# egordm/tch-geometric

Measured on AMD Instinct MI355X. Metric: sampled edges/sec, neighbor_sampling_homogenous fanout [15,10] on RMAT-24, higher is better.
Workload: dtype int64

## Files before the change

include/tchgeo.h:

```cpp
#ifndef TCHGEO_H
#define TCHGEO_H

#include <stdint.h>

#ifdef __cplusplus
extern "C" {
#endif

#define TG_API __attribute__((visibility("default")))

#define TG_OK 0
#define TG_ERR_INVALID 1
#define TG_ERR_HIP 2
#define TG_ERR_UNSUPPORTED 3

#define TG_MAX_HOPS 8
#define TG_MAX_FANOUT 32

typedef struct {
    const int64_t *ptrs;
    const int64_t *indices;
    const double *weights;
    const int64_t *timestamps;
    int64_t n_major;
// ... 71 lines not shown

TG_API int tg_ns_homo_batched_form(const tg_graph *csc, int64_t n_batches, int64_t n_seeds, const int64_t *fanout,
                            int32_t n_hops, const tg_ns_config *cfg, const tg_ns_out *out, int64_t workspace_bytes,
                            int32_t mode, int32_t *form, int32_t *n_windows);

TG_API int tg_ns_homo_batched_pipeline(const tg_graph *csc, int64_t n_batches, int64_t n_seeds, const int64_t *fanout,
                                int32_t n_hops, const tg_ns_config *cfg, const tg_ns_out *out, int64_t workspace_bytes,
                                int32_t mode, int32_t *staged);

typedef struct {
    int64_t window_bytes;
    int32_t gather_blocks;
    int32_t gather_threads;
    int32_t emit_threads;
    int32_t direct_hop0;
    int32_t fuse_first_hops;
    int32_t fold_hist;
    int32_t emit_blocks;
    int32_t staged;
    int32_t stage_round_chunks;
    int32_t stage_gather_threads;
    int32_t stage_gather_blocks;
    int32_t stage_emit_threads;
    int32_t stage_parts;
    int32_t stage_part_min_batches;
    int32_t stage_sort_blocks;
    int32_t stage_fine;
    int32_t stage_concurrent;
    int32_t stage_split;
    int32_t stage_split_round_chunks;
    int32_t store_align64;
    int32_t stage_fine_sub_bits;
    int32_t stage_fine_blocks;
} tg_ns_win_tuning;
TG_API int tg_ns_win_tuning_get(tg_ns_win_tuning *t);
TG_API int tg_ns_win_tuning_set(const tg_ns_win_tuning *t);

TG_API int tg_ns_win_stage_timing(int32_t enable);
TG_API int tg_ns_win_stage_times(float *ms, char *names, int32_t cap, int32_t *n);

typedef struct {
    const int64_t *vertices;
    const int64_t *ids;
    const int64_t *call_ids;
    int64_t m;
    int64_t id_base;
    int32_t fanout;
    int32_t sampler;
    uint32_t rng_tag;
    uint32_t _reserved;
} tg_hop_in;

typedef struct {
    int64_t *cnt;
    int64_t *offsets;
    int64_t *neighbors;
    int64_t *edge_ptrs;
    int64_t *parents;
} tg_hop_out;

TG_API int tg_ns_hop_workspace_bytes(int64_t m, int64_t *bytes);
TG_API int tg_ns_hop(const tg_graph *csc, const tg_hop_in *in, const tg_rng *rng, const tg_hop_out *out,
                     void *workspace, int64_t workspace_bytes, void *stream);

typedef struct {
    int32_t filter_mode;
// ... 293 lines not shown
```

tch-geometric_amd/csrc/ns_homo_win.hip:

```cpp
#include <stdlib.h>

#include <algorithm>
#include <mutex>

#include "ns_tickets.h"
#include "stage_bits.h"
#include "tg_device.h"
#include "tg_host.h"

namespace tg {

constexpr int WIN_PART_BLOCKS = 512;
constexpr int WIN_PART_THREADS = 512;
constexpr int WIN_TILE = 4096;
constexpr int WIN_MAX_BUCKETS = 8192;
constexpr int WIN_MAX_ROWS = 1024;
constexpr int WIN_MAX_PARTS = 16;

struct WinState {
    int64_t begin, end, ne, fbase;
};

struct WinQueues {
    struct alignas(256) Q {
// ... 8 lines not shown
    const uint32_t *ptrs32;
    const int64_t *seeds;
    int64_t n_seeds, n_batches;
    int32_t n_hops, hop, k, kmax;
    int64_t cap_nodes, cap_edges;
    int64_t *samples, *rows, *cols, *edge_index, *layer_offsets, *counts;
    uint64_t seed, call_id;
    uint32_t tag;
    int64_t id_base;
    WinState *state;
    CallKey *call_keys;
    unsigned long long *n_items;
    void *items_in, *items_sorted;
    uint32_t *hist;
    uint32_t *base;
    WinQueues *queues;
    int32_t n_buckets, shift;
    int32_t slot_bits;
    int32_t n_rows;
    int64_t item_pitch;
    uint32_t *vtab;
    uint32_t *stage;
    int32_t n_windows, idx_bits, next_idx_bits;
    int32_t n_wbuckets;
    uint32_t store_align;
    void *items_fine;
    uint16_t *item_keys;
    uint32_t *fine_rowtot;
    uint32_t *fine_tot, *fine_start;
    uint32_t *fine_tile_off;
    int64_t next_pitch;
    int64_t b0;
    int32_t fine_sub_bits;
    TG_BOUNDS_FIELDS
};

struct WinItemN {
    uint32_t e0, deg, bs, e;
    __device__ __forceinline__ static WinItemN make(uint64_t e0, uint32_t deg, uint32_t b, uint32_t slot, uint32_t e,
                                                    int slot_bits) {
        return WinItemN{(uint32_t)e0, deg, (b << slot_bits) | slot, e};
    }
    __device__ __forceinline__ uint64_t col() const { return e0; }
    __device__ __forceinline__ uint32_t batch(int slot_bits) const { return bs >> slot_bits; }
    __device__ __forceinline__ uint32_t slot(int slot_bits) const { return bs & ((1u << slot_bits) - 1u); }
};
struct WinItemW {
    uint64_t e0;
    uint32_t deg, b, s, e;
    __device__ __forceinline__ static WinItemW make(uint64_t e0, uint32_t deg, uint32_t b, uint32_t slot, uint32_t e,
                                                    int) {
        return WinItemW{e0, deg, b, slot, e};
    }
    __device__ __forceinline__ uint64_t col() const { return e0; }
    __device__ __forceinline__ uint32_t batch(int) const { return b; }
    __device__ __forceinline__ uint32_t slot(int) const { return s; }
};
static_assert(sizeof(WinItemN) == 16 && sizeof(WinItemW) == 24, "item layouts");

__device__ __forceinline__ uint32_t win_bucket(uint64_t e0, int shift, int n_buckets) {
    const uint32_t w = (uint32_t)(e0 >> shift);
    return (w & 7u) * (uint32_t)(n_buckets >> 3) + (w >> 3);
}

__global__ void win_init_kernel(const WinParams p, int64_t n_batches) {
    const int64_t b = blockIdx.x;
    int64_t *samples = p.samples + b * p.cap_nodes;
    for (int64_t i = threadIdx.x; i < p.n_seeds; i += blockDim.x) samples[i] = p.seeds[b * p.n_seeds + i];
    if (threadIdx.x == 0) {
        p.state[b] = WinState{0, p.n_seeds, 0, 0};
        p.call_keys[b] = call_key(p.seed, p.call_id + (uint64_t)b, p.tag);
        if (p.n_hops == 0) {
            p.counts[b * 2 + 0] = p.n_seeds;
            p.counts[b * 2 + 1] = 0;
        }
        if (b == 0)
            for (int h = 0; h < TG_MAX_HOPS; ++h) p.n_items[h] = 0ull;
    }
}

constexpr int WIN_ROUND_CHUNKS = 32;
constexpr int WIN_EMIT_MAX_THREADS = 512;
constexpr int WIN_STAGE_FIRST_RC = 16;
constexpr int WIN_STAGE_SIDE_RC = 8;

__host__ __device__ inline size_t win_emit_wave_lds_bytes(int kmax) {
    return (size_t)64 * kmax * sizeof(uint32_t) + (((size_t)64 * kmax + 15) & ~(size_t)15) + 64;
}

__host__ __device__ inline size_t win_emit_head_bytes(int rc = WIN_ROUND_CHUNKS) {
    return (((size_t)(rc + 1) * sizeof(uint32_t) + 15) & ~(size_t)15) + 16 +
           (size_t)rc * 64 * (sizeof(int64_t) + sizeof(uint32_t));
}
__host__ __device__ inline size_t win_emit_lds_bytes(int kmax, int n_waves, int rc = WIN_ROUND_CHUNKS) {
    return win_emit_head_bytes(rc) + (size_t)n_waves * win_emit_wave_lds_bytes(kmax);
}

__device__ __forceinline__ void win_next_item(const WinParams &p, int64_t b, uint32_t rel, uint32_t v, uint32_t *lhist);

template <typename Item, int KMAX, bool REPLACE, bool DIRECT, bool FOLD = false, bool NEXT = false, bool ITEMS = true,
          int RC = WIN_ROUND_CHUNKS>
__device__ __forceinline__ WinState win_emit_hop(const WinParams &p, unsigned char *smem, const int64_t b, const int hop,
                                                 const int k, const WinState st, const CallKey ck,
                                                 uint32_t *lhist = nullptr) {
    const int tid = threadIdx.x, lane = tid & 63, wave = tid >> 6, n_waves = blockDim.x >> 6;
    uint32_t *chunk_off = reinterpret_cast<uint32_t *>(smem);
    constexpr int64_t ROUND_SLOTS = (int64_t)RC * 64;
    const size_t off_bytes = (((size_t)(RC + 1) * sizeof(uint32_t)) + 15) & ~(size_t)15;
    int64_t *shared_fbase = reinterpret_cast<int64_t *>(smem + off_bytes);
    int64_t *col0 = reinterpret_cast<int64_t *>(smem + off_bytes + 16);
    uint32_t *cdeg = reinterpret_cast<uint32_t *>(smem + off_bytes + 16 + (size_t)ROUND_SLOTS * sizeof(int64_t));
    unsigned char *wbase = smem + win_emit_head_bytes(RC) + (size_t)wave * win_emit_wave_lds_bytes(p.kmax);
    uint32_t *spos = reinterpret_cast<uint32_t *>(wbase);
    uint8_t *slane = wbase + (size_t)64 * p.kmax * sizeof(uint32_t);
    Item *items = static_cast<Item *>(p.items_in);

    int64_t *samples = p.samples + b * p.cap_nodes;
    int64_t *rows = p.rows + b * p.cap_edges;
    int64_t *cols = p.cols + b * p.cap_edges;
    int64_t *eidx = p.edge_index + b * p.cap_edges;
    const int64_t n_seeds = p.n_seeds;
    const int64_t begin = st.begin, end = st.end;
    int64_t ne = st.ne;

    if (tid == 0) {
        int64_t *lo = p.layer_offsets + (b * p.n_hops + hop) * 3;
        lo[0] = n_seeds + ne;
        lo[1] = ne;
        lo[2] = n_seeds + ne;
        if (!FOLD) *shared_fbase = (DIRECT || !ITEMS) ? 0 : (int64_t)atomicAdd(&p.n_items[hop], (unsigned long long)(end - begin));
    }
    if (!FOLD) __syncthreads();
    const int64_t fbase = FOLD ? b * p.item_pitch : *shared_fbase;

    for (int64_t round_begin = begin; round_begin < end; round_begin += ROUND_SLOTS) {
        const int64_t round_end = min(end, round_begin + ROUND_SLOTS);
        const int nc = (int)((round_end - round_begin + 63) >> 6);
        for (int c = wave; c < nc; c += n_waves) {
            const int64_t i = round_begin + (int64_t)c * 64 + lane;
            int64_t e0 = 0, deg = 0;
            if (i < round_end) {
                int64_t w = samples[i];
                TG_CHECK_VERTEX(p, w);
                if (p.ptrs32) {
                    e0 = (int64_t)p.ptrs32[w];
                    deg = (int64_t)p.ptrs32[w + 1] - e0;
                } else {
                    e0 = p.ptrs[w];
                    deg = p.ptrs[w + 1] - e0;
                }
            }
            col0[c * 64 + lane] = e0;
            cdeg[c * 64 + lane] = deg > 0 ? (uint32_t)deg : 0u;
            const uint32_t cnt = (deg <= 0) ? 0u : (REPLACE ? (uint32_t)k : (uint32_t)min(deg, (int64_t)k));
            const uint32_t tot = wave_sum(cnt);
            if (lane == 0) chunk_off[c] = tot;
        }
        __syncthreads();
        if (wave == 0) {
            const uint32_t v = lane < nc ? chunk_off[lane] : 0u;
            const uint32_t incl = wave_inclusive_scan(v);
            if (lane < nc) chunk_off[lane] = incl - v;
            if (lane == 63) chunk_off[nc] = incl;
        }
        __syncthreads();
        for (int c = wave; c < nc; c += n_waves) {
            const int64_t i0 = round_begin + (int64_t)c * 64;
            const int64_t i = i0 + lane;
            const int64_t e0 = col0[c * 64 + lane];
            const uint32_t n = cdeg[c * 64 + lane];
            const uint32_t cnt = (n == 0) ? 0u : (REPLACE ? (uint32_t)k : min(n, (uint32_t)k));
            const uint64_t did = (uint64_t)(p.id_base + i);
            const uint32_t incl = wave_inclusive_scan(cnt);
            const uint32_t excl = incl - cnt;
            const uint32_t total = __shfl(incl, 63, 64);
            const int64_t e_chunk = ne + (int64_t)chunk_off[c];
            if (!DIRECT && ITEMS && i < round_end) {
                items[fbase + (i - begin)] =
                    Item::make((uint64_t)e0, n, (uint32_t)b, (uint32_t)i, (uint32_t)(e_chunk + excl), p.slot_bits);
                if (FOLD && n) atomicAdd(&lhist[win_bucket((uint64_t)e0, p.shift, p.n_buckets)], 1u);
            }
            const bool draws = REPLACE ? (cnt > 0) : (n > (uint32_t)k);
            const uint64_t dmask = __ballot(draws);
            const int n_draw = __popcll(dmask);
            const bool spread = n_draw > 0 && n_draw <= 32;
            if (spread) {
                uint8_t *dl = slane + (((size_t)64 * p.kmax + 15) & ~(size_t)15);
                const int my_rank = __popcll(dmask & ((lane == 0) ? 0ull : (~0ull >> (64 - lane))));
                if (draws) dl[my_rank] = (uint8_t)lane;
// ... 48 lines not shown
                    }
                } else {
                    sample_tickets<KMAX>(ck, did, n, k, spos, slane, excl, lane);
                }
            }
            wave_lds_handoff();
            if constexpr (DIRECT) {
                for (uint32_t q0 = 0; q0 < total; q0 += 256) {
                    int l4[4];
                    int64_t ep[4], v[4];
#pragma unroll
                    for (int u = 0; u < 4; ++u) {
                        const uint32_t q = q0 + (uint32_t)(u * 64 + lane);
                        const uint32_t qq = q < total ? q : 0u;
                        l4[u] = slane[qq];
                        ep[u] = col0[c * 64 + l4[u]] + (int64_t)spos[qq];
                    }
                    if (p.indices32) {
#pragma unroll
                        for (int u = 0; u < 4; ++u) v[u] = (int64_t)__builtin_nontemporal_load(&p.indices32[ep[u]]);
                    } else {
#pragma unroll
                        for (int u = 0; u < 4; ++u) v[u] = __builtin_nontemporal_load(&p.indices[ep[u]]);
                    }
#pragma unroll
                    for (int u = 0; u < 4; ++u) {
                        const uint32_t q = q0 + (uint32_t)(u * 64 + lane);
                        if (q < total) {
                            const int64_t e = e_chunk + q;
                            samples[n_seeds + e] = v[u];
                            __builtin_nontemporal_store(n_seeds + e, &rows[e]);
                            __builtin_nontemporal_store(i0 + (int64_t)l4[u], &cols[e]);
                            __builtin_nontemporal_store(ep[u], &eidx[e]);
                            if (NEXT) win_next_item(p, b, (uint32_t)(n_seeds + e - end), (uint32_t)v[u], lhist);
                        }
                    }
                }
            } else
            {
                typedef long long i64x2 __attribute__((ext_vector_type(2)));
                const int64_t ea = e_chunk;
                const uint32_t am = p.store_align;
                const uint32_t head_r = (uint32_t)((am + 1u - (uint32_t)(((uintptr_t)(rows + ea) >> 3) & am)) & am);
                const uint32_t head_c = (uint32_t)((am + 1u - (uint32_t)(((uintptr_t)(cols + ea) >> 3) & am)) & am);
                const uint32_t head_e = (uint32_t)((am + 1u - (uint32_t)(((uintptr_t)(eidx + ea) >> 3) & am)) & am);
                if ((uint32_t)lane < total) {
                    if ((uint32_t)lane < head_r) __builtin_nontemporal_store(n_seeds + ea + (int64_t)lane, &rows[ea + lane]);
                    if ((uint32_t)lane < head_c) __builtin_nontemporal_store(i0 + (int64_t)slane[lane], &cols[ea + lane]);
                    if ((uint32_t)lane < head_e)
                        __builtin_nontemporal_store(col0[c * 64 + slane[lane]] + (int64_t)spos[lane], &eidx[ea + lane]);
                }
                for (uint32_t q = head_r + 2u * lane; q < total; q += 128) {
                    const int64_t e = ea + q;
                    if (q + 1 < total) {
                        i64x2 r = {n_seeds + e, n_seeds + e + 1};
                        __builtin_nontemporal_store(r, reinterpret_cast<i64x2 *>(&rows[e]));
                    } else
                        __builtin_nontemporal_store(n_seeds + e, &rows[e]);
                }
                for (uint32_t q = head_c + 2u * lane; q < total; q += 128) {
                    const int64_t e = ea + q;
                    if (q + 1 < total) {
                        i64x2 cc = {i0 + (int64_t)slane[q], i0 + (int64_t)slane[q + 1]};
                        __builtin_nontemporal_store(cc, reinterpret_cast<i64x2 *>(&cols[e]));
                    } else
                        __builtin_nontemporal_store(i0 + (int64_t)slane[q], &cols[e]);
                }
// ... 301 lines not shown
        const uint32_t cnt = (n == 0) ? 0u : (REPLACE ? (uint32_t)k : min(n, (uint32_t)k));
        const uint32_t incl = wave_inclusive_scan(cnt);
        const uint32_t excl = incl - cnt;
        const uint32_t total = __shfl(incl, 63, 64);
        if (cnt > 0) {
            const uint32_t b = it.batch(p.slot_bits);
            const CallKey ck = p.call_keys[b];
            const uint64_t did = (uint64_t)(p.id_base + (int64_t)it.slot(p.slot_bits));
            ebase[lane] = (int64_t)it.col();
            obase[lane] = (int64_t)b * p.cap_nodes + p.n_seeds + (int64_t)it.e - (int64_t)excl;
            if (REPLACE) {
                sample_replace_any(ck, did, n, k, spos, slane, excl, lane);
            } else if (n <= (uint32_t)k) {
                for (uint32_t s = 0; s < cnt; ++s) {
                    spos[excl + s] = s;
                    slane[excl + s] = (uint8_t)lane;
                }
            } else {
                sample_tickets<KMAX>(ck, did, n, k, spos, slane, excl, lane);
            }
        }
        wave_lds_handoff();
        if (p.indices32)
            win_gather_chunk<uint32_t>(p.indices32, total, lane, slane, spos, ebase, obase, p.samples);
        else
            win_gather_chunk<int64_t>(p.indices, total, lane, slane, spos, ebase, obase, p.samples);
        if (tid == 0) slice_lo[buf ^ 1] = nxt;
        __syncthreads();
    }
}

#include "ns_homo_stage.inl"

__device__ __forceinline__ void win_next_item(const WinParams &p, int64_t b, uint32_t rel, uint32_t v, uint32_t *lhist) {
    static_cast<WinItem8 *>(p.items_in)[b * p.next_pitch + rel] = WinItem8{v, ((uint32_t)b << p.next_idx_bits) | rel};
    if (lhist) {
        const uint32_t c = win_stage_key(lhist + p.n_buckets, p.n_windows, p.n_wbuckets, v, 4).coarse;
        atomicAdd(&lhist[c], 1u);
        p.item_keys[b * p.next_pitch + rel] = (uint16_t)c;
    }
}

static int win_env_int(const char *name, int dflt) {
    const char *v = getenv(name);
    return v ? atoi(v) : dflt;
}

struct WinTuning {
    int64_t window_bytes;
    int32_t gather_blocks, gather_threads, emit_threads, direct_hop0, fuse_first_hops, fold_hist, emit_blocks;
    int32_t staged, stage_round_chunks, stage_gather_threads, stage_gather_blocks, stage_emit_threads, stage_parts, stage_part_min_batches, stage_sort_blocks;
    int32_t stage_fine, stage_concurrent, stage_split, stage_split_round_chunks, store_align64, stage_fine_sub_bits, stage_fine_blocks;
};
static WinTuning &win_tuning() {
    static WinTuning t = {
        (int64_t)win_env_int("TG_WIN_KIB", 512) * 1024,
        win_env_int("TG_WIN_GATHER_BLOCKS", 256),
        win_env_int("TG_WIN_GATHER_THREADS", 512),
        win_env_int("TG_WIN_EMIT_THREADS", 256),
        win_env_int("TG_WIN_DIRECT_HOP0", 1),
        win_env_int("TG_WIN_FUSE_FIRST_HOPS", 1),
        win_env_int("TG_WIN_FOLD_HIST", 1),
        win_env_int("TG_WIN_EMIT_BLOCKS", 768),
        win_env_int("TG_WIN_STAGED", 2),
        win_env_int("TG_WIN_STAGE_ROUND_CHUNKS", 2),
        win_env_int("TG_WIN_STAGE_GATHER_THREADS", 512),
        win_env_int("TG_WIN_STAGE_GATHER_BLOCKS", 512),
        win_env_int("TG_WIN_STAGE_EMIT_THREADS", 256),
        win_env_int("TG_WIN_STAGE_PARTS", 1),
        win_env_int("TG_WIN_STAGE_PART_MIN_BATCHES", 1024),
        win_env_int("TG_WIN_STAGE_SORT_BLOCKS", 768),
        win_env_int("TG_WIN_STAGE_FINE", 1),
        win_env_int("TG_WIN_STAGE_CONCURRENT", 0),
        win_env_int("TG_WIN_STAGE_SPLIT", 0),
        win_env_int("TG_WIN_STAGE_SPLIT_ROUND_CHUNKS", 4),
        win_env_int("TG_WIN_STORE_ALIGN64", 1),
        win_env_int("TG_WIN_STAGE_FINE_SUB_BITS", 7),
        win_env_int("TG_WIN_STAGE_FINE_BLOCKS", 2048),
    };
    return t;
}

constexpr int WIN_MAX_STAGES = 8 * TG_MAX_HOPS + 2;
struct WinStageClock {
    bool enabled = false;
    int n = 0;
    hipEvent_t ev[WIN_MAX_STAGES + 1] = {};
    char name[WIN_MAX_STAGES][24] = {};
    void begin(hipStream_t s) {
        n = 0;
        if (!enabled) return;
        if (!ev[0])
            for (auto &e : ev) (void)hipEventCreate(&e);
        (void)hipEventRecord(ev[0], s);
    }
    void mark(const char *what, int hop, hipStream_t s) {
        if (!enabled || n >= WIN_MAX_STAGES) return;
        snprintf(name[n], sizeof(name[n]), "%s.h%d", what, hop);
        ++n;
        (void)hipEventRecord(ev[n], s);
    }
};
static WinStageClock &win_clock() {
    static WinStageClock c;
    return c;
}

struct WinLayout {
    size_t state, call_keys, n_items, queues, hist, base, items_in, items_sorted, vtab, fine_tot, fine_start, fine_tile_off, item_keys, stage, total, total_push;
    int64_t max_items;
    int stage_words;
};

static StageBits win_stage_bits(const tg_graph *csc) {
    StageBits sb;
    if (!csc) {
        sb.bv = sb.bp = 32;
        return sb;
    }
    sb.bv = stage_bits_of((uint64_t)std::max<int64_t>(csc->n_major, 1) - 1);
    const int64_t longest = csc->max_degree > 0 ? csc->max_degree : csc->n_edges;
    sb.bp = stage_bits_of((uint64_t)std::max<int64_t>(longest, 1) - 1);
    return sb;
}
static int win_stage_words(const tg_graph *csc, const int64_t *fanout, int32_t n_hops) {
    int64_t k = 0;
    for (int h = 1; h < n_hops; ++h) k = std::max(k, fanout[h]);
    if (n_hops < 2 || k > 32) return 0;
    if (!csc) return 32;
    const int bits = stage_slot_bits((int)k, win_stage_bits(csc));
    return (bits <= 512 && k <= 16) ? 16 : (bits <= 1024 ? 32 : 0);
}

static WinLayout win_layout(const tg_graph *csc, int64_t n_batches, int64_t n_seeds, const int64_t *fanout, int32_t n_hops) {
    WinLayout L;
    int64_t layer = n_seeds, widest = n_seeds;
    for (int h = 0; h + 1 < n_hops; ++h) {
        layer *= fanout[h];
        if (layer > widest) widest = layer;
    }
    L.max_items = n_batches * widest;
    size_t at = 0;
    auto take = [&](size_t bytes) {
        const size_t here = at;
        at += (bytes + 255) & ~(size_t)255;
        return here;
    };
    L.state = take((size_t)n_batches * sizeof(WinState));
    L.call_keys = take((size_t)n_batches * sizeof(CallKey));
    L.n_items = take(TG_MAX_HOPS * sizeof(unsigned long long));
    L.queues = take(WIN_MAX_PARTS * sizeof(WinQueues));
    L.hist = take((size_t)std::max(WIN_MAX_ROWS, WIN_MAX_PARTS * WIN_PART_BLOCKS) * WIN_MAX_BUCKETS * sizeof(uint32_t));
    L.base = take((size_t)WIN_MAX_PARTS * (WIN_MAX_BUCKETS + 8) * sizeof(uint32_t));
    L.items_in = take((size_t)L.max_items * sizeof(WinItemW));
    L.items_sorted = take((size_t)L.max_items * sizeof(WinItemW));
    L.vtab = take((size_t)(WIN_MAX_BUCKETS + 8) * sizeof(uint32_t));
    L.total_push = at;
    L.fine_tot = take((size_t)WIN_MAX_PARTS * (WIN_MAX_BUCKETS / 8 + 8) * WIN_FINE_PER_COARSE_MAX * sizeof(uint32_t));
    L.fine_start = take((size_t)WIN_MAX_PARTS * (WIN_MAX_BUCKETS / 8 + 8) * WIN_FINE_PER_COARSE_MAX * sizeof(uint32_t));
    L.fine_tile_off = take(((size_t)L.max_items / WIN_FINE_TILE + WIN_MAX_PARTS + 1) * WIN_FINE_BINS_MAX * sizeof(uint32_t));
    L.item_keys = take((size_t)L.max_items * sizeof(uint16_t));
    L.stage_words = win_stage_words(csc, fanout, n_hops);
    L.stage = take((size_t)L.max_items * L.stage_words * sizeof(uint32_t));
    L.total = at;
    return L;
}

template <typename Item, int KMAX, bool REPLACE>
static int win_run(WinParams p, int64_t n_batches, const int64_t *fanout, int32_t n_hops, hipStream_t stream) {
    const WinTuning t = win_tuning();
    WinStageClock &clk = win_clock();
    const int gather_blocks = (t.gather_blocks + 7) & ~7;
    const bool fold = t.fold_hist && t.direct_hop0 && t.fuse_first_hops && n_hops > 1;
    const size_t hist_lds = fold ? (size_t)p.n_buckets * sizeof(uint32_t) : 0;
    auto emit_threads_for = [&]() {
        int threads = t.emit_threads;
        while (threads > 64 && win_emit_lds_bytes(p.kmax, threads / 64) + hist_lds > 64 * 1024)
            threads = ((threads >> 1) + 63) & ~63;
        return threads;
    };
    p.n_batches = n_batches;
    p.n_rows = (int32_t)std::min<int64_t>(std::min(std::max(t.emit_blocks, 1), WIN_MAX_ROWS), n_batches);
    auto pitch_of = [&](int h) {
        int64_t f = p.n_seeds;
        for (int j = 0; j < h; ++j) f *= fanout[j];
        return f;
    };
    clk.begin(stream);
    int h0 = 0;
// ... 118 lines not shown
    p.n_windows = (int32_t)((csc->n_edges >> p.shift) + 1);
    auto pitch_of = [&](int h) {
        int64_t f = p.n_seeds;
        for (int j = 0; j < h; ++j) f *= fanout[j];
        return f;
    };
    auto bits_of = [&](int64_t pitch) {
        int bits = 1;
        while (((int64_t)1 << bits) < pitch) ++bits;
        return bits;
    };
    p.n_wbuckets = (p.n_buckets + 63) & ~63;
    p.n_buckets = p.n_wbuckets >> 3;
    const size_t tables = win_stage_tables_bytes(p.n_buckets, p.n_windows);
    int parts = std::min(std::max(t.stage_parts, 1), WIN_MAX_PARTS);
    while (parts > 1 && n_batches / parts < std::max(t.stage_part_min_batches, 1)) --parts;
    if (clk.enabled) parts = 1;
    const bool split = t.stage_split && !clk.enabled;
    if (split) parts = 1;
    WinSide &side = win_side();
    std::unique_lock<std::mutex> side_lock(side.mu, std::defer_lock);
    if (parts > 1 || split) {
        side_lock.lock();
        const int rc = side.ensure();
        if (rc != TG_OK) return rc;
    }
    uint32_t *const hist0 = p.hist, *const base0 = p.base;
    WinQueues *const queues0 = p.queues;
    void *const sorted0 = p.items_sorted, *const in0 = p.items_in;
    uint32_t *const fine_tot0 = p.fine_tot, *const fine_start0 = p.fine_start, *const fine_tile_off0 = p.fine_tile_off;
    const bool first_in_parts = parts > 1 && n_hops == 2;

    int fthreads = std::min(t.emit_threads, WIN_EMIT_MAX_THREADS);
    while (fthreads > 64 && win_emit_lds_bytes(p.kmax, fthreads / 64, WIN_STAGE_FIRST_RC) + tables > 64 * 1024)
        fthreads = ((fthreads >> 1) + 63) & ~63;
    auto rows_of = [&](int64_t nb) {
        return (int32_t)std::min<int64_t>(std::min(std::max(t.stage_sort_blocks, 1), WIN_MAX_ROWS), nb);
    };
    auto part_tables = [&](int part) {
        p.hist = hist0 + (size_t)part * WIN_MAX_ROWS * (WIN_MAX_BUCKETS / 8);
        p.base = base0 + (size_t)part * (WIN_MAX_BUCKETS + 8);
        p.queues = queues0 + part;
    };
    auto launch_first = [&](int part, int64_t b0, int64_t nb, hipStream_t ps) {
        part_tables(part);
        p.b0 = b0;
        p.n_batches = nb;
        p.n_rows = rows_of(nb);
        p.next_pitch = pitch_of(1);
        p.next_idx_bits = bits_of(p.next_pitch);
        hipLaunchKernelGGL((win_stage_first_kernel<KFIRST, REPLACE>), dim3((unsigned)p.n_rows), dim3(fthreads),
                           win_emit_lds_bytes(p.kmax, fthreads / 64, WIN_STAGE_FIRST_RC) + tables, ps, p, (int)fanout[0]);
    };
    const bool concurrent = first_in_parts && t.stage_concurrent;

    clk.begin(stream);
    hipLaunchKernelGGL(win_vtab_kernel, dim3((p.n_windows + 256) / 256), dim3(256), 0, stream, p, csc->n_major);
    TG_LAUNCH_CHECK();
    if (!first_in_parts) {
        launch_first(0, 0, n_batches, stream);
        TG_LAUNCH_CHECK();
        clk.mark("first", 0, stream);
    }
    if (concurrent) {
        TG_HIP(hipEventRecord(side.gathered[0], stream));
        TG_HIP(hipStreamWaitEvent(side.stream, side.gathered[0], 0));
    }
    for (int h = 1; h < n_hops; ++h) {
        const bool next = h + 1 < n_hops;
        const int hparts = next ? 1 : parts;
        for (int part = 0; part < hparts; ++part) {
            const int64_t b0 = n_batches * part / hparts, nb = n_batches * (part + 1) / hparts - b0;
            const bool counted = h == 1 && (first_in_parts || hparts == 1);
            hipStream_t ps = (concurrent && (part & 1)) ? side.stream : stream;
            if (first_in_parts) {
                launch_first(part, b0, nb, ps);
                TG_LAUNCH_CHECK();
            }
            p.hop = h;
            p.k = (int32_t)fanout[h];
            p.item_pitch = pitch_of(h);
            p.idx_bits = bits_of(p.item_pitch);
            p.next_pitch = next ? pitch_of(h + 1) : 0;
            p.next_idx_bits = next ? bits_of(p.next_pitch) : 0;
            int ethreads = t.stage_emit_threads;
            int rc = std::min(std::max(split ? t.stage_split_round_chunks : t.stage_round_chunks, 1), WIN_STAGE_ROUND_CHUNKS_MAX);
            while (win_stage_emit_lds_bytes(W, p.k, ethreads / 64, rc, split) > 64 * 1024) {
                if (rc > 1)
                    rc >>= 1;
                else if (ethreads > 64)
                    ethreads = ((ethreads >> 1) + 63) & ~63;
// ... 210 lines not shown
    p.kmax = 1;
    for (int h = 0; h < n_hops; ++h) p.kmax = fanout[h] > p.kmax ? (int32_t)fanout[h] : p.kmax;
    p.cap_nodes = out->cap_nodes;
    p.cap_edges = out->cap_edges;
    p.samples = out->samples;
    p.rows = out->rows;
    p.cols = out->cols;
    p.edge_index = out->edge_index;
    p.layer_offsets = out->layer_offsets;
    p.counts = out->counts;
    p.seed = rng->seed;
    p.call_id = rng->call_id;
    p.tag = (cfg && cfg->rng_tag) ? cfg->rng_tag : TG_TAG_NS_HOMO;
    p.id_base = cfg ? cfg->id_base : 0;
    TG_BOUNDS_INIT(p, csc);
    unsigned char *w = static_cast<unsigned char *>(ws);
    p.state = reinterpret_cast<WinState *>(w + L.state);
    p.call_keys = reinterpret_cast<CallKey *>(w + L.call_keys);
    p.n_items = reinterpret_cast<unsigned long long *>(w + L.n_items);
    p.queues = reinterpret_cast<WinQueues *>(w + L.queues);
    p.hist = reinterpret_cast<uint32_t *>(w + L.hist);
    p.base = reinterpret_cast<uint32_t *>(w + L.base);
    p.items_in = w + L.items_in;
    p.items_sorted = w + L.items_sorted;
    win_window_geometry(csc, &p.shift, &p.n_buckets);
    int slot_bits = 1;
    while (((int64_t)1 << slot_bits) < out->cap_nodes) ++slot_bits;
    const bool narrow = csc->n_edges < ((int64_t)1 << 32) && out->cap_edges < ((int64_t)1 << 32) && slot_bits < 32 &&
                        n_batches <= ((int64_t)1 << (32 - slot_bits));
    const bool force_wide = mode == TG_NS_FORM_WINDOWED_WIDE;
    p.slot_bits = slot_bits;
    const bool repl = (cfg ? cfg->sampler : TG_SAMPLER_UNIFORM) == TG_SAMPLER_UNIFORM_REPL;
    p.vtab = reinterpret_cast<uint32_t *>(w + L.vtab);
    p.fine_tot = reinterpret_cast<uint32_t *>(w + L.fine_tot);
    p.fine_start = reinterpret_cast<uint32_t *>(w + L.fine_start);
    p.fine_tile_off = reinterpret_cast<uint32_t *>(w + L.fine_tile_off);
    p.item_keys = reinterpret_cast<uint16_t *>(w + L.item_keys);
    p.stage = reinterpret_cast<uint32_t *>(w + L.stage);
    if (narrow && !force_wide && ws_bytes >= (int64_t)L.total &&
        win_staged_applicable(p, win_tuning(), csc, n_batches, fanout, n_hops, L.stage_words))
        return repl ? win_dispatch_staged<true>(p, csc, L.stage_words, n_batches, fanout, n_hops, stream)
                    : win_dispatch_staged<false>(p, csc, L.stage_words, n_batches, fanout, n_hops, stream);
    if (narrow && !force_wide) return win_dispatch<WinItemN>(p, repl, n_batches, fanout, n_hops, stream);
    return win_dispatch<WinItemW>(p, repl, n_batches, fanout, n_hops, stream);
}

extern "C" int tg_ns_win_tuning_get(tg_ns_win_tuning *t) {
    TG_REQUIRE(t, "tg_ns_win_tuning_get: null");
    const tg::WinTuning &w = tg::win_tuning();
    t->window_bytes = w.window_bytes;
    t->gather_blocks = w.gather_blocks;
    t->gather_threads = w.gather_threads;
    t->emit_threads = w.emit_threads;
    t->direct_hop0 = w.direct_hop0;
    t->fuse_first_hops = w.fuse_first_hops;
    t->fold_hist = w.fold_hist;
    t->emit_blocks = w.emit_blocks;
    t->staged = w.staged;
    t->stage_round_chunks = w.stage_round_chunks;
    t->stage_gather_threads = w.stage_gather_threads;
    t->stage_gather_blocks = w.stage_gather_blocks;
    t->stage_emit_threads = w.stage_emit_threads;
    t->stage_parts = w.stage_parts;
    t->stage_part_min_batches = w.stage_part_min_batches;
    t->stage_sort_blocks = w.stage_sort_blocks;
    t->stage_fine = w.stage_fine;
    t->stage_concurrent = w.stage_concurrent;
    t->stage_split = w.stage_split;
    t->stage_split_round_chunks = w.stage_split_round_chunks;
    t->store_align64 = w.store_align64;
    t->stage_fine_sub_bits = w.stage_fine_sub_bits;
    t->stage_fine_blocks = w.stage_fine_blocks;
    return TG_OK;
}

extern "C" int tg_ns_win_tuning_set(const tg_ns_win_tuning *t) {
    TG_REQUIRE(t, "tg_ns_win_tuning_set: null");
    TG_REQUIRE(t->window_bytes == 0 || (t->window_bytes >= 64 && t->window_bytes <= ((int64_t)1 << 32)),
               "tg_ns_win_tuning_set: window_bytes outside [64, 2^32]");
    TG_REQUIRE(t->gather_threads == 0 || (t->gather_threads >= 64 && t->gather_threads <= 1024 && t->gather_threads % 64 == 0),
               "tg_ns_win_tuning_set: gather_threads must be a multiple of 64 in [64, 1024]");
    TG_REQUIRE(t->emit_threads == 0 || (t->emit_threads >= 64 && t->emit_threads <= 1024 && t->emit_threads % 64 == 0),
               "tg_ns_win_tuning_set: emit_threads must be a multiple of 64 in [64, 1024]");
    TG_REQUIRE(t->gather_blocks >= 0 && t->gather_blocks <= 65536, "tg_ns_win_tuning_set: gather_blocks outside [0, 65536]");
    tg::WinTuning &w = tg::win_tuning();
    if (t->window_bytes) w.window_bytes = t->window_bytes;
    if (t->gather_blocks) w.gather_blocks = t->gather_blocks;
    if (t->gather_threads) w.gather_threads = t->gather_threads;
    if (t->emit_threads) w.emit_threads = t->emit_threads;
    if (t->direct_hop0 >= 0) w.direct_hop0 = t->direct_hop0 != 0;
    if (t->fuse_first_hops >= 0) w.fuse_first_hops = t->fuse_first_hops != 0;
    if (t->fold_hist >= 0) w.fold_hist = t->fold_hist != 0;
    if (t->emit_blocks > 0) w.emit_blocks = t->emit_blocks;
    if (t->staged >= 0) w.staged = t->staged > 2 ? 1 : t->staged;
    if (t->stage_round_chunks > 0) w.stage_round_chunks = t->stage_round_chunks;
    if (t->stage_gather_threads >= 64 && t->stage_gather_threads <= 1024) w.stage_gather_threads = t->stage_gather_threads & ~63;
    if (t->stage_gather_blocks > 0) w.stage_gather_blocks = t->stage_gather_blocks;
    if (t->stage_emit_threads >= 64 && t->stage_emit_threads <= 1024) w.stage_emit_threads = t->stage_emit_threads & ~63;
    if (t->stage_parts > 0) w.stage_parts = t->stage_parts;
    if (t->stage_part_min_batches > 0) w.stage_part_min_batches = t->stage_part_min_batches;
    if (t->stage_sort_blocks > 0) w.stage_sort_blocks = t->stage_sort_blocks;
    if (t->stage_fine >= 0) w.stage_fine = t->stage_fine != 0;
    if (t->stage_concurrent >= 0) w.stage_concurrent = t->stage_concurrent != 0;
    if (t->stage_split >= 0) w.stage_split = t->stage_split != 0;
    if (t->stage_split_round_chunks > 0) w.stage_split_round_chunks = t->stage_split_round_chunks;
    if (t->store_align64 >= 0) w.store_align64 = t->store_align64 != 0;
    if (t->stage_fine_sub_bits > 0) w.stage_fine_sub_bits = std::min(std::max(t->stage_fine_sub_bits, 4), tg::WIN_FINE_SUB_BITS_MAX);
    if (t->stage_fine_blocks > 0) w.stage_fine_blocks = std::min((t->stage_fine_blocks + 7) & ~7, 8192);
    return TG_OK;
}

extern "C" int tg_ns_win_stage_timing(int32_t enable) {
    tg::win_clock().enabled = enable != 0;
    return TG_OK;
}

extern "C" int tg_ns_win_stage_times(float *ms, char *names, int32_t cap, int32_t *n) {
    TG_REQUIRE(n && (cap == 0 || (ms && names)), "tg_ns_win_stage_times: null arguments");
    tg::WinStageClock &c = tg::win_clock();
    *n = c.n;
    if (c.n == 0) return TG_OK;
    TG_HIP(hipEventSynchronize(c.ev[c.n]));
    for (int i = 0; i < c.n && i < cap; ++i) {
        TG_HIP(hipEventElapsedTime(&ms[i], c.ev[i], c.ev[i + 1]));
        snprintf(names + (size_t)i * 24, 24, "%s", c.name[i]);
    }
    return TG_OK;
}

extern "C" int tg_ns_homo_batched_form(const tg_graph *csc, int64_t n_batches, int64_t n_seeds, const int64_t *fanout,
                                       int32_t n_hops, const tg_ns_config *cfg, const tg_ns_out *out,
                                       int64_t workspace_bytes, int32_t mode, int32_t *form, int32_t *n_windows) {
    TG_REQUIRE(csc && out && form && (fanout || n_hops == 0), "tg_ns_homo_batched_form: null arguments");
    TG_REQUIRE(n_hops >= 0 && n_hops <= TG_MAX_HOPS, "tg_ns_homo_batched_form: n_hops %d outside [0, %d]", n_hops, TG_MAX_HOPS);
    *form = TG_NS_FORM_FUSED;
    if (n_windows) *n_windows = 0;
    const int sampler = cfg ? cfg->sampler : TG_SAMPLER_UNIFORM;
    const int filter = cfg ? cfg->filter_mode : TG_FILTER_NONE;
    if (sampler == TG_SAMPLER_WEIGHTED || filter != TG_FILTER_NONE) return TG_OK;
    if (workspace_bytes <= 0 || !tg_ns_homo_windowed_applicable(csc, n_batches, n_seeds, fanout, n_hops, cfg, out, mode))
        return TG_OK;
// ... 28 lines not shown
```

tch-geometric_amd/tch_geometric/_cabi.py:

```python
import ctypes as C
import os

import torch

_HERE = os.path.dirname(os.path.abspath(__file__))
LIB_PATH = os.environ.get("TCHGEO_LIB") or os.path.join(os.path.dirname(_HERE), "lib", "libtchgeo_hip.so")

TG_OK = 0
TG_MAX_HOPS = 8
TG_MAX_FANOUT = 32
SAMPLER_UNIFORM, SAMPLER_UNIFORM_REPL, SAMPLER_WEIGHTED = 0, 1, 2
PART_REPLY_PACKED, PART_REPLY_PAIRS, PART_REPLY_TRIPLES, PART_REPLY_PACKED_STATE = 1, 2, 3, 4
FILTER_NONE, FILTER_STATIC, FILTER_RELATIVE, FILTER_DYNAMIC = -1, 0, 1, 2

EXPORTS = ["tg_version", "tg_last_error", "tg_ns_homo_capacity", "tg_ns_homo_batched", "tg_random_walk",
           "tg_edge_set_bytes", "tg_edge_set_build", "tg_random_walk_es",
           "tg_tempo_random_walk", "tg_rmat_edges", "tg_seed_batches", "tg_ind2ptr", "tg_probe_random_gather",
           "tg_neg_workspace_bytes", "tg_neg_sample", "tg_hgt_workspace_bytes", "tg_hgt_sample", "tg_ns_hop_workspace_bytes", "tg_ns_hop", "tg_rmat_edges_rect",
           "tg_coo_to_csx_workspace_bytes", "tg_coo_to_csx", "tg_budget_layer", "tg_check_range",
           "tg_ns_hop_scan_workspace_bytes", "tg_ns_hop_scan", "tg_ns_hop_weighted", "tg_ns_hop_weighted_groups", "tg_ns_hop_weighted_workspace_bytes", "tg_gather_rows",
           "tg_biased_walk_workspace_bytes", "tg_biased_tempo_random_walk", "tg_ns_hetero_capacity",
           "tg_ns_hetero_batched", "tg_ns_homo_compact", "tg_part_workspace_bytes", "tg_part_begin",
           "tg_sanitize_range", "tg_ns_hop_segments", "tg_het_hop_begin_all", "tg_het_hop_end_all", "tg_part_requests", "tg_part_count", "tg_part_scan_workspace_bytes", "tg_part_sample", "tg_part_emit", "tg_part_slot_words", "tg_part_sample_slots", "tg_part_emit_slots", "tg_part_unpack", "tg_part_pack", "tg_compact_rows", "tg_budget_capacity",
           "tg_budget_workspace_bytes", "tg_budget_sample", "tg_ns_homo_workspace_bytes", "tg_ns_homo_batched_ws", "tg_het_meta_words", "tg_het_step_begin",
# ... 192 lines not shown
    cfg.sampler, cfg.filter_mode = sampler, filter_mode
    fan = (C.c_int64 * max(len(fanout), 1))(*fanout)
    so = out.struct()
    taken, n_win = C.c_int32(0), C.c_int32(0)
    check(lib.tg_ns_homo_batched_form(C.byref(graph), C.c_int64(n_batches), C.c_int64(n_seeds), fan,
                                      C.c_int32(len(fanout)), C.byref(cfg), C.byref(so),
                                      C.c_int64(ws.numel() * 8 if ws is not None else 0), C.c_int32(form),
                                      C.byref(taken), C.byref(n_win)))
    return taken.value, n_win.value


def ns_homo_batched_staged(graph, out, n_batches, n_seeds, fanout, ws=None, form=0, sampler=SAMPLER_UNIFORM):
    cfg = TgNsConfig()
    cfg.sampler, cfg.filter_mode = sampler, FILTER_NONE
    fan = (C.c_int64 * max(len(fanout), 1))(*fanout)
    so = out.struct()
    st = C.c_int32(0)
    check(lib.tg_ns_homo_batched_pipeline(C.byref(graph), C.c_int64(n_batches), C.c_int64(n_seeds), fan,
                                          C.c_int32(len(fanout)), C.byref(cfg), C.byref(so),
                                          C.c_int64(ws.numel() * 8 if ws is not None else 0), C.c_int32(form), C.byref(st)))
    return bool(st.value)


class TgNsWinTuning(C.Structure):
    _fields_ = [("window_bytes", C.c_int64), ("gather_blocks", C.c_int32), ("gather_threads", C.c_int32),
                ("emit_threads", C.c_int32), ("direct_hop0", C.c_int32), ("fuse_first_hops", C.c_int32),
                ("fold_hist", C.c_int32), ("emit_blocks", C.c_int32), ("staged", C.c_int32),
                ("stage_round_chunks", C.c_int32), ("stage_gather_threads", C.c_int32), ("stage_gather_blocks", C.c_int32),
                ("stage_emit_threads", C.c_int32), ("stage_parts", C.c_int32),
                ("stage_part_min_batches", C.c_int32), ("stage_sort_blocks", C.c_int32), ("stage_fine", C.c_int32),
                ("stage_concurrent", C.c_int32), ("stage_split", C.c_int32),
                ("stage_split_round_chunks", C.c_int32), ("store_align64", C.c_int32),
                ("stage_fine_sub_bits", C.c_int32),
                ("stage_fine_blocks", C.c_int32)]


def ns_win_tuning():
    t = TgNsWinTuning()
    check(lib.tg_ns_win_tuning_get(C.byref(t)))
    return {k: getattr(t, k) for k, _ in TgNsWinTuning._fields_}


def ns_win_tuning_set(**kw):
    before = ns_win_tuning()
    t = TgNsWinTuning(0, 0, 0, 0, -1, -1, -1, 0, -1, 0, 0, 0, 0, 0, 0, 0, -1, -1, -1, 0, -1, 0, 0)
    for k, v in kw.items():
        assert k in before, k
        setattr(t, k, int(v))
    check(lib.tg_ns_win_tuning_set(C.byref(t)))
    return before


def ns_win_stage_timing(enable):
    check(lib.tg_ns_win_stage_timing(C.c_int32(int(bool(enable)))))


def ns_win_stage_times():
    cap = 80
    ms, names, n = (C.c_float * cap)(), C.create_string_buffer(24 * cap), C.c_int32(0)
    check(lib.tg_ns_win_stage_times(ms, names, C.c_int32(cap), C.byref(n)))
    return [(names.raw[24 * i:24 * i + 24].split(b"\0", 1)[0].decode(), float(ms[i])) for i in range(min(n.value, cap))]


def edge_set(graph, device):
    nbytes = C.c_int64(0)
    check(lib.tg_edge_set_bytes(C.byref(graph), C.byref(nbytes)))
    es = torch.empty(nbytes.value // 8, dtype=torch.int64, device=device)
    check(lib.tg_edge_set_build(C.byref(graph), ptr(es), nbytes, stream_ptr(device)))
    return es


def random_walk(graph, start, walk_length, p, q, seed, call_id, edge_set=None):
    walks = torch.empty((start.numel(), walk_length + 1), dtype=torch.int64, device=start.device)
    rng = TgRng(seed, call_id)
    if edge_set is None:
        check(lib.tg_random_walk(C.byref(graph), ptr(start), C.c_int64(start.numel()), C.c_int64(walk_length),
                                 C.c_float(p), C.c_float(q), C.byref(rng), ptr(walks), stream_ptr(start.device)))
    else:
# ... 280 lines not shown
```

Measured before the change: 71.23 billion.

## Add lean first-hop stage kernel with vertex index table and seed prefetch

Adds a stage_first tuning mode, on by default. It builds a coarse vertex-index table (vidx) so the window/bucket key lookup in the next-item path can jump straight into the window table instead of searching it. The first-hop kernel reads seeds directly, with several chunks' CSR bounds loads in flight at once, and can use a pipelined variant with prefetched bounds. The aim is to cut the latency of the first-hop bounds gathers and the cost of per-item key lookups. In exchange it adds an extra kernel launch, more LDS table space, and device code in files not shown here (win_stage_key_idx, the pipe kernel, win_vidx_kernel).

```diff
diff --git a/include/tchgeo.h b/include/tchgeo.h
--- a/include/tchgeo.h
+++ b/include/tchgeo.h
@@ -127,6 +127,7 @@
     int32_t store_align64;
     int32_t stage_fine_sub_bits;
     int32_t stage_fine_blocks;
+    int32_t stage_first;
 } tg_ns_win_tuning;
 TG_API int tg_ns_win_tuning_get(tg_ns_win_tuning *t);
 TG_API int tg_ns_win_tuning_set(const tg_ns_win_tuning *t);
diff --git a/tch-geometric_amd/csrc/ns_homo_win.hip b/tch-geometric_amd/csrc/ns_homo_win.hip
--- a/tch-geometric_amd/csrc/ns_homo_win.hip
+++ b/tch-geometric_amd/csrc/ns_homo_win.hip
@@ -64,6 +64,8 @@
     int64_t next_pitch;
     int64_t b0;
     int32_t fine_sub_bits;
+    uint16_t *vidx;
+    int32_t vidx_shift, n_vidx;
     TG_BOUNDS_FIELDS
 };
 
@@ -128,13 +130,19 @@
     return win_emit_head_bytes(rc) + (size_t)n_waves * win_emit_wave_lds_bytes(kmax);
 }
 
+template <bool VIDX>
 __device__ __forceinline__ void win_next_item(const WinParams &p, int64_t b, uint32_t rel, uint32_t v, uint32_t *lhist);
 
+template <int PF>
+struct WinPre {
+    uint32_t e0[PF > 0 ? PF : 1], deg[PF > 0 ? PF : 1];
+};
+
 template <typename Item, int KMAX, bool REPLACE, bool DIRECT, bool FOLD = false, bool NEXT = false, bool ITEMS = true,
-          int RC = WIN_ROUND_CHUNKS>
+          int RC = WIN_ROUND_CHUNKS, int PF = 0, bool VIDX = false, bool SEEDS = false>
 __device__ __forceinline__ WinState win_emit_hop(const WinParams &p, unsigned char *smem, const int64_t b, const int hop,
                                                  const int k, const WinState st, const CallKey ck,
-                                                 uint32_t *lhist = nullptr) {
+                                                 uint32_t *lhist = nullptr, const WinPre<PF> *pre = nullptr) {
     const int tid = threadIdx.x, lane = tid & 63, wave = tid >> 6, n_waves = blockDim.x >> 6;
     uint32_t *chunk_off = reinterpret_cast<uint32_t *>(smem);
     constexpr int64_t ROUND_SLOTS = (int64_t)RC * 64;
@@ -168,25 +176,59 @@
     for (int64_t round_begin = begin; round_begin < end; round_begin += ROUND_SLOTS) {
         const int64_t round_end = min(end, round_begin + ROUND_SLOTS);
         const int nc = (int)((round_end - round_begin + 63) >> 6);
-        for (int c = wave; c < nc; c += n_waves) {
-            const int64_t i = round_begin + (int64_t)c * 64 + lane;
-            int64_t e0 = 0, deg = 0;
-            if (i < round_end) {
-                int64_t w = samples[i];
-                TG_CHECK_VERTEX(p, w);
-                if (p.ptrs32) {
-                    e0 = (int64_t)p.ptrs32[w];
-                    deg = (int64_t)p.ptrs32[w + 1] - e0;
-                } else {
-                    e0 = p.ptrs[w];
-                    deg = p.ptrs[w + 1] - e0;
-                }
-            }
+        auto pass_a = [&](int c, int64_t e0, int64_t deg) {
             col0[c * 64 + lane] = e0;
             cdeg[c * 64 + lane] = deg > 0 ? (uint32_t)deg : 0u;
             const uint32_t cnt = (deg <= 0) ? 0u : (REPLACE ? (uint32_t)k : (uint32_t)min(deg, (int64_t)k));
             const uint32_t tot = wave_sum(cnt);
             if (lane == 0) chunk_off[c] = tot;
+        };
+        if constexpr (PF > 0) {
+#pragma unroll
+            for (int u = 0; u < PF; ++u)
+                if (wave + u * n_waves < nc) pass_a(wave + u * n_waves, (int64_t)pre->e0[u], (int64_t)pre->deg[u]);
+        } else {
+            auto bounds = [&](int c, int64_t &e0, int64_t &deg) {
+                const int64_t i = round_begin + (int64_t)c * 64 + lane;
+                e0 = 0;
+                deg = 0;
+                if (i < round_end) {
+                    int64_t w;
+                    if constexpr (SEEDS) {
+                        w = p.seeds[b * n_seeds + i];
+                        samples[i] = w;
+                    } else
+                        w = samples[i];
+                    TG_CHECK_VERTEX(p, w);
+                    if (p.ptrs32) {
+                        e0 = (int64_t)p.ptrs32[w];
+                        deg = (int64_t)p.ptrs32[w + 1] - e0;
+                    } else {
+                        e0 = p.ptrs[w];
+                        deg = p.ptrs[w + 1] - e0;
+                    }
+                }
+            };
+            if constexpr (SEEDS) {
+                constexpr int U = 4;
+                for (int c0 = wave; c0 < nc; c0 += U * n_waves) {
+                    int64_t e0[U], deg[U];
+#pragma unroll
+                    for (int u = 0; u < U; ++u) {
+                        e0[u] = 0;
+                        deg[u] = 0;
+                        if (c0 + u * n_waves < nc) bounds(c0 + u * n_waves, e0[u], deg[u]);
+                    }
+#pragma unroll
+                    for (int u = 0; u < U; ++u)
+                        if (c0 + u * n_waves < nc) pass_a(c0 + u * n_waves, e0[u], deg[u]);
+                }
+            } else
+                for (int c = wave; c < nc; c += n_waves) {
+                    int64_t e0, deg;
+                    bounds(c, e0, deg);
+                    pass_a(c, e0, deg);
+                }
         }
         __syncthreads();
         if (wave == 0) {
@@ -301,7 +343,7 @@
                             __builtin_nontemporal_store(n_seeds + e, &rows[e]);
                             __builtin_nontemporal_store(i0 + (int64_t)l4[u], &cols[e]);
                             __builtin_nontemporal_store(ep[u], &eidx[e]);
-                            if (NEXT) win_next_item(p, b, (uint32_t)(n_seeds + e - end), (uint32_t)v[u], lhist);
+                            if (NEXT) win_next_item<VIDX>(p, b, (uint32_t)(n_seeds + e - end), (uint32_t)v[u], lhist);
                         }
                     }
                 }
@@ -669,10 +711,14 @@
 
 #include "ns_homo_stage.inl"
 
+template <bool VIDX>
 __device__ __forceinline__ void win_next_item(const WinParams &p, int64_t b, uint32_t rel, uint32_t v, uint32_t *lhist) {
     static_cast<WinItem8 *>(p.items_in)[b * p.next_pitch + rel] = WinItem8{v, ((uint32_t)b << p.next_idx_bits) | rel};
     if (lhist) {
-        const uint32_t c = win_stage_key(lhist + p.n_buckets, p.n_windows, p.n_wbuckets, v, 4).coarse;
+        const uint32_t *lvtab = lhist + p.n_buckets;
+        const uint32_t c = VIDX ? win_stage_key_idx(lvtab, win_stage_lvidx(lhist, p.n_buckets, p.n_windows), p.vidx_shift,
+                                                    p.n_vidx, p.n_wbuckets, v, 4).coarse
+                                : win_stage_key(lvtab, p.n_windows, p.n_wbuckets, v, 4).coarse;
         atomicAdd(&lhist[c], 1u);
         p.item_keys[b * p.next_pitch + rel] = (uint16_t)c;
     }
@@ -688,6 +734,7 @@
     int32_t gather_blocks, gather_threads, emit_threads, direct_hop0, fuse_first_hops, fold_hist, emit_blocks;
     int32_t staged, stage_round_chunks, stage_gather_threads, stage_gather_blocks, stage_emit_threads, stage_parts, stage_part_min_batches, stage_sort_blocks;
     int32_t stage_fine, stage_concurrent, stage_split, stage_split_round_chunks, store_align64, stage_fine_sub_bits, stage_fine_blocks;
+    int32_t stage_first;
 };
 static WinTuning &win_tuning() {
     static WinTuning t = {
@@ -714,6 +761,7 @@
         win_env_int("TG_WIN_STORE_ALIGN64", 1),
         win_env_int("TG_WIN_STAGE_FINE_SUB_BITS", 7),
         win_env_int("TG_WIN_STAGE_FINE_BLOCKS", 2048),
+        win_env_int("TG_WIN_STAGE_FIRST", 1),
     };
     return t;
 }
@@ -744,7 +792,7 @@
 }
 
 struct WinLayout {
-    size_t state, call_keys, n_items, queues, hist, base, items_in, items_sorted, vtab, fine_tot, fine_start, fine_tile_off, item_keys, stage, total, total_push;
+    size_t state, call_keys, n_items, queues, hist, base, items_in, items_sorted, vtab, vidx, fine_tot, fine_start, fine_tile_off, item_keys, stage, total, total_push;
     int64_t max_items;
     int stage_words;
 };
@@ -792,6 +840,7 @@
     L.items_in = take((size_t)L.max_items * sizeof(WinItemW));
     L.items_sorted = take((size_t)L.max_items * sizeof(WinItemW));
     L.vtab = take((size_t)(WIN_MAX_BUCKETS + 8) * sizeof(uint32_t));
+    L.vidx = take(win_vidx_bytes());
     L.total_push = at;
     L.fine_tot = take((size_t)WIN_MAX_PARTS * (WIN_MAX_BUCKETS / 8 + 8) * WIN_FINE_PER_COARSE_MAX * sizeof(uint32_t));
     L.fine_start = take((size_t)WIN_MAX_PARTS * (WIN_MAX_BUCKETS / 8 + 8) * WIN_FINE_PER_COARSE_MAX * sizeof(uint32_t));
@@ -976,8 +1025,17 @@
     const bool first_in_parts = parts > 1 && n_hops == 2;
 
     int fthreads = std::min(t.emit_threads, WIN_EMIT_MAX_THREADS);
-    while (fthreads > 64 && win_emit_lds_bytes(p.kmax, fthreads / 64, WIN_STAGE_FIRST_RC) + tables > 64 * 1024)
+    const size_t ftables = t.stage_first ? win_stage_first_tables_bytes(p.n_buckets, p.n_windows) : tables;
+    while (fthreads > 64 && win_emit_lds_bytes(p.kmax, fthreads / 64, WIN_STAGE_FIRST_RC) + ftables > 64 * 1024)
         fthreads = ((fthreads >> 1) + 63) & ~63;
+    const bool first_pipe = t.stage_first == 2 && p.n_seeds <= (int64_t)64 * std::min(WIN_STAGE_FIRST_RC, WIN_FIRST_PF * (fthreads / 64));
+    const bool first_lean = t.stage_first && !first_pipe;
+    if (t.stage_first) {
+        const int64_t nm = std::max<int64_t>(csc->n_major, 1);
+        p.vidx_shift = 0;
+        while (((nm - 1) >> p.vidx_shift) >= WIN_VIDX_MAX) ++p.vidx_shift;
+        p.n_vidx = (int32_t)(((nm - 1) >> p.vidx_shift) + 1);
+    }
     auto rows_of = [&](int64_t nb) {
         return (int32_t)std::min<int64_t>(std::min(std::max(t.stage_sort_blocks, 1), WIN_MAX_ROWS), nb);
     };
@@ -993,14 +1051,25 @@
         p.n_rows = rows_of(nb);
         p.next_pitch = pitch_of(1);
         p.next_idx_bits = bits_of(p.next_pitch);
-        hipLaunchKernelGGL((win_stage_first_kernel<KFIRST, REPLACE>), dim3((unsigned)p.n_rows), dim3(fthreads),
-                           win_emit_lds_bytes(p.kmax, fthreads / 64, WIN_STAGE_FIRST_RC) + tables, ps, p, (int)fanout[0]);
+        if (first_pipe)
+            hipLaunchKernelGGL((win_stage_first_pipe_kernel<KFIRST, REPLACE>), dim3((unsigned)p.n_rows), dim3(fthreads),
+                               win_emit_lds_bytes(p.kmax, fthreads / 64, WIN_STAGE_FIRST_RC) + ftables, ps, p, (int)fanout[0]);
+        else if (first_lean)
+            hipLaunchKernelGGL((win_stage_first_kernel<KFIRST, REPLACE, true>), dim3((unsigned)p.n_rows), dim3(fthreads),
+                               win_emit_lds_bytes(p.kmax, fthreads / 64, WIN_STAGE_FIRST_RC) + ftables, ps, p, (int)fanout[0]);
+        else
+            hipLaunchKernelGGL((win_stage_first_kernel<KFIRST, REPLACE, false>), dim3((unsigned)p.n_rows), dim3(fthreads),
+                               win_emit_lds_bytes(p.kmax, fthreads / 64, WIN_STAGE_FIRST_RC) + tables, ps, p, (int)fanout[0]);
     };
     const bool concurrent = first_in_parts && t.stage_concurrent;
 
     clk.begin(stream);
     hipLaunchKernelGGL(win_vtab_kernel, dim3((p.n_windows + 256) / 256), dim3(256), 0, stream, p, csc->n_major);
     TG_LAUNCH_CHECK();
+    if (t.stage_first) {
+        hipLaunchKernelGGL(win_vidx_kernel, dim3((p.n_vidx + 256) / 256), dim3(256), 0, stream, p);
+        TG_LAUNCH_CHECK();
+    }
     if (!first_in_parts) {
         launch_first(0, 0, n_batches, stream);
         TG_LAUNCH_CHECK();
@@ -1277,6 +1346,7 @@
     p.slot_bits = slot_bits;
     const bool repl = (cfg ? cfg->sampler : TG_SAMPLER_UNIFORM) == TG_SAMPLER_UNIFORM_REPL;
     p.vtab = reinterpret_cast<uint32_t *>(w + L.vtab);
+    p.vidx = reinterpret_cast<uint16_t *>(w + L.vidx);
     p.fine_tot = reinterpret_cast<uint32_t *>(w + L.fine_tot);
     p.fine_start = reinterpret_cast<uint32_t *>(w + L.fine_start);
     p.fine_tile_off = reinterpret_cast<uint32_t *>(w + L.fine_tile_off);
@@ -1316,6 +1386,7 @@
     t->store_align64 = w.store_align64;
     t->stage_fine_sub_bits = w.stage_fine_sub_bits;
     t->stage_fine_blocks = w.stage_fine_blocks;
+    t->stage_first = w.stage_first;
     return TG_OK;
 }
 
@@ -1352,6 +1423,7 @@
     if (t->store_align64 >= 0) w.store_align64 = t->store_align64 != 0;
     if (t->stage_fine_sub_bits > 0) w.stage_fine_sub_bits = std::min(std::max(t->stage_fine_sub_bits, 4), tg::WIN_FINE_SUB_BITS_MAX);
     if (t->stage_fine_blocks > 0) w.stage_fine_blocks = std::min((t->stage_fine_blocks + 7) & ~7, 8192);
+    if (t->stage_first >= 0) w.stage_first = std::min(t->stage_first, 2);
     return TG_OK;
 }
 
diff --git a/tch-geometric_amd/tch_geometric/_cabi.py b/tch-geometric_amd/tch_geometric/_cabi.py
--- a/tch-geometric_amd/tch_geometric/_cabi.py
+++ b/tch-geometric_amd/tch_geometric/_cabi.py
@@ -248,7 +248,7 @@
                 ("stage_concurrent", C.c_int32), ("stage_split", C.c_int32),
                 ("stage_split_round_chunks", C.c_int32), ("store_align64", C.c_int32),
                 ("stage_fine_sub_bits", C.c_int32),
-                ("stage_fine_blocks", C.c_int32)]
+                ("stage_fine_blocks", C.c_int32), ("stage_first", C.c_int32)]
 
 
 def ns_win_tuning():
@@ -259,7 +259,7 @@
 
 def ns_win_tuning_set(**kw):
     before = ns_win_tuning()
-    t = TgNsWinTuning(0, 0, 0, 0, -1, -1, -1, 0, -1, 0, 0, 0, 0, 0, 0, 0, -1, -1, -1, 0, -1, 0, 0)
+    t = TgNsWinTuning(0, 0, 0, 0, -1, -1, -1, 0, -1, 0, 0, 0, 0, 0, 0, 0, -1, -1, -1, 0, -1, 0, 0, -1)
     for k, v in kw.items():
         assert k in before, k
         setattr(t, k, int(v))
```

After: 71.85 billion, median of 6. Within noise of the previous version (+0.9%).
